# szemenyeim/DynEnv

Measured on AMD Instinct MI355X. Metric: agent-steps/s, higher is better.
Workload: dtype f64

## Files before the change

dynenv_amd/csrc/driving_dev.h:

```cpp
#pragma once
#include "dev_common.h"

#define DRV_MAXA 10
#define DRV_MAXP 20
#define DRV_MAXO 20
#define DRV_NB 32
#define DRV_NS 24
#define DRV_SLOT_PED 10
#define DRV_SLOT_OBST 30
#define DRV_SLOT_BLD 50
#define DRV_W 1700.0
#define DRV_H 1000.0
#define DRV_MAX_TIME 6000
#define DRV_TIME_DIFF 10
#define DRV_LANE_ROWS 8

enum { BF_PX = 0, BF_PY, BF_VX, BF_VY, BF_ANG, BF_W, BF_VBX, BF_VBY, BF_WB, BF_COUNT };
enum { CF_DIRX = 0, CF_DIRY, CF_PREVX, CF_PREVY, CF_GOALX, CF_GOALY, CF_COUNT };
enum { EI_ELAPSED = 0, EI_ALLFIN, EI_NPED, EI_NOBST, EI_EPISODE, EI_OCC, EI_ERR, EI_PAD,
       EI_N_FAST, EI_N_QUIET, EI_N_CONTACT, EI_N_SLOTS,
       EI_N_WHY_CAND, EI_N_WHY_MOVING, EI_N_WHY_INERT, EI_N_STEADY, EI_N_LIGHT,
       EI_N_SPLIT,
       EI_DEFER_OBS,
       EI_COUNT };
// ... 3 lines not shown
#define CARF_TYPE(f) ((f)&3)
#define CARF_TEAM(f) (((f) >> 2) & 3)
#define CARF_PACK(type, team, fin, crashed, fric, lp) \
  ((type) | ((team) << 2) | ((fin) << 4) | ((crashed) << 5) | ((fric) << 6) | ((lp) << 8))
#define PEDF_PACK(road, side, dead, crossing, begin, speed) \
  ((road) | ((side) << 1) | ((dead) << 2) | ((crossing) << 3) | ((begin) << 4) | ((speed) << 8))

struct DrvRoad {
  int nLanes;
  double width, length, dirAngle, followDist;
  double cosDir0;
  V2 p0, p1, dir, normal;
  V2 walk[2][2];
};

struct DrvConst {
  DrvRoad roads[2];
  float laneRows[DRV_LANE_ROWS * 5];
  double carMass[4], carInertia[4], carHx[4], carHy[4], carPower[4];
  double pedMass, pedInertia;
  double turnCos[2], turnSin[2];
};

struct PvIn {
  double px, py, ang;
  double ox, oy;
  double gx, gy;
  int flags;
};

struct DrvState {
  int E, A, obs_dim, pad0;
  uint64_t seed;
  int env_id_offset, pad1;
  double* body;
  double* carx;
  int* flags;
  int* aux;
  double* obst;
  int* envi;
  double* epr;
  int* s_pair;
  int* s_meta;
  uint32_t* s_hash;
  double* s_imp;
  int* lastcand;
  int* iso;
  int* iso_done;
  unsigned* iso_hw;
  int* pvq;
  int pv_par;
  int tick, iso_on;
  int tick_src;
};
#ifndef DRV_ISO_MAX
#define DRV_ISO_MAX 192
#endif
#ifndef DRV_ISO_MIN_E
#define DRV_ISO_MIN_E 3072
#endif
#define DRV_ISO_LIST 256
#define DRV_ISO_HDR 16
#define DRV_ISO_WORDS (DRV_ISO_HDR + 3 * DRV_ISO_LIST)
#define DRV_ISO_COOLDOWN 64
#define DRV_ISO_G0 256
#define DRV_ISO_GSPAN 256
#define DRV_ISO_GROUPS 1024
// ... 1 lines not shown
```

dynenv_amd/csrc/driving_kernels.hip:

```cpp
#include "driving_dev.h"

__constant__ DrvConst C;

#include "driving_host.h"

struct DrvMailbox {
  double p1x[DRV_NS][2], p1y[DRV_NS][2], p2x[DRV_NS][2], p2y[DRV_NS][2], nx[DRV_NS], ny[DRV_NS];
  int hash[DRV_NS][2], count[DRV_NS], flag[DRV_NS];
};
struct DrvObsStage {
  float carRow[DRV_MAXA][8];
  float goal[DRV_MAXA][2];
  float shared[DRV_MAXO * 4 + DRV_MAXP * 2 + DRV_LANE_ROWS * 5];
};
#ifdef DRV_PROFILE
#define DRV_PROF(...) __VA_ARGS__
#else
#define DRV_PROF(...)
#endif
#define DRV_CLIST 128
struct __align__(16) DrvLds {
  double px[DRV_NB], py[DRV_NB], vx[DRV_NB], vy[DRV_NB], ang[DRV_NB], w[DRV_NB], vbx[DRV_NB], vby[DRV_NB], wb[DRV_NB];
  double minv[DRV_NB], iinv[DRV_NB];
  double rc[16], rs[16], rotAng[16];
  double dirx[16], diry[16], prevx[16], prevy[16], goalx[16], goaly[16];
  double cosRel0[16];
  double dprev[16];
  double cmass[16], cpower[16], chx[16], chy[16];
  double aabb[DRV_MAXA][4];
  int flags[DRV_NB], moving[DRV_NB];
  double ox[DRV_MAXO], oy[DRV_MAXO];
  int s_pair[DRV_NS], s_meta[DRV_NS], s_hash0[DRV_NS], s_hash1[DRV_NS];
  double s_jn0[DRV_NS], s_jt0[DRV_NS], s_jn1[DRV_NS], s_jt1[DRV_NS];
  double rewAcc[16], posAcc[16];
  int lastCand[64];
  int stepErr;
  unsigned char act[16];
  int still[DRV_NB];
  unsigned short clist[DRV_CLIST];
  int clistN;
  int sLvMeta;
  unsigned long long sActive;
  unsigned char sLevel[DRV_NS];
  union {
    DrvMailbox mb;
    DrvObsStage ob;
  } u;
};

static_assert(sizeof(DrvLds) <= 10240, "16 one-wave workgroups per CU - one residency round of 4096 environments on 256 CUs - need <= 160 KB / 16 of LDS each");
__shared__ DrvLds g_L;


#define CF_FIN(f) (((f) >> 4) & 1)
#define CF_CRASHED(f) (((f) >> 5) & 1)
#define CF_FRIC(f) (((f) >> 6) & 1)
#define CF_LP(f) (((f) >> 8) & 7)
#define CF_SET_LP(f, lp) (((f) & ~(7 << 8)) | ((lp) << 8))
#define CF_CRASH_BITS ((1 << 4) | (1 << 5) | (1 << 6))
#define PF_ROAD(f) ((f)&1)
#define PF_SIDE(f) (((f) >> 1) & 1)
#define PF_DEAD(f) (((f) >> 2) & 1)
#define PF_CROSSING(f) (((f) >> 3) & 1)
#define PF_BEGIN(f) (((f) >> 4) & 1)
#define PF_SPEED(f) (((f) >> 8) & 15)

#define DRV_COS_PI_2 6.123233995736766e-17
template <int R>
struct RoadK;
template <>
struct RoadK<0> {
  static constexpr double p0x = 875.0, p0y = 0.0, dirx = 0.0, diry = 1.0, lat = 2.0 * 35.0 + 5.0, length = 1000.0;
  static constexpr double dirAngle = 1.5707963267948966, cosDir0 = DRV_COS_PI_2, nx = -1.0, ny = DRV_COS_PI_2;
};
// ... 556 lines not shown
      apply_impulse(a, vneg(jj), r1[c]);
      apply_impulse(b, jj, r2[c]);
    }
  }
}

DE_DEV bool arb_apply_bias_only(BodyV& a, BodyV& b, V2 n, const V2* r1, const V2* r2, const double* nMass, const double* bias,
                                double* jBias, int count) {
  bool changed = false;
#define DRV_BIAS_PASS(c)                                              \
  {                                                                   \
    double vbn = bias_rel_n(a, b, r1[c], r2[c], n);                   \
    double jbnOld = jBias[c];                                         \
    jBias[c] = dms_acc_clamp0(bias[c] - vbn, nMass[c], jbnOld);       \
    changed |= jBias[c] != jbnOld;                                    \
    V2 jb = vmul(n, jBias[c] - jbnOld);                               \
    apply_bias_impulse(a, vneg(jb), r1[c]);                           \
    apply_bias_impulse(b, jb, r2[c]);                                 \
  }
  DRV_BIAS_PASS(0)
  if (count > 1) DRV_BIAS_PASS(1)
#undef DRV_BIAS_PASS
  return changed;
}
DE_DEV bool arb_is_bias_only(const BodyV& a, const BodyV& b, const double* jn, const double* jt, const double* bounce, int count) {
  long long z = __double_as_longlong(a.v.x) | __double_as_longlong(a.v.y) | __double_as_longlong(a.w) |
                __double_as_longlong(b.v.x) | __double_as_longlong(b.v.y) | __double_as_longlong(b.w);
  bool ok = true;
#pragma unroll
  for (int c = 0; c < 2; ++c)
    if (c == 0 || count > 1) { z |= __double_as_longlong(jn[c]) | __double_as_longlong(jt[c]); ok = ok && bounce[c] == 0.0; }
  return ok && z == 0ll;
}
DE_DEV void body_load_bias(const DrvLds& L, int idx, BodyV& b) {
  if (idx < DRV_SLOT_OBST) { b.vb = v2(L.vbx[idx], L.vby[idx]); b.wb = L.wb[idx]; }
}
DE_DEV void body_store_bias(DrvLds& L, int idx, const BodyV& b) {
  if (idx < DRV_SLOT_OBST) { L.vbx[idx] = b.vb.x; L.vby[idx] = b.vb.y; L.wb[idx] = b.wb; }
}
#define DRV_ZERO_SLOT 30
#define DRV_SINK_SLOT 31
static_assert(DRV_SLOT_OBST == DRV_ZERO_SLOT && DRV_NB == 32, "body slots 30 and 31 are free");
DE_DEV int body_rd(int idx) { return idx < DRV_SLOT_OBST ? idx : DRV_ZERO_SLOT; }
DE_DEV int body_wr(int idx) { return idx < DRV_SLOT_OBST ? idx : DRV_SINK_SLOT; }

struct DrvSplitRet { double jn0, jn1, jb0, jb1, jt0, jt1; int pk, pair, bits; };
DE_OOL DrvSplitRet drv_solve_general_split(int lane, int myLevel_, int bodyAB, int lvl_, double nMass0, double nMass1, double bias0, double bias1,
                                           double bounce0, double bounce1, double jn0, double jn1, double jt0, double jt1, int pk, int pair,
                                           int bits3) {
  DrvLds& L = g_L;
  DrvMailbox& M = L.u.mb;
  int code = ((pk >> 30) & 1) | (((pk >> 8) & 0xFF) << 1) | (myLevel_ << 8);
  const int maxLevel = (int)(signed char)(uniform_i(lvl_) & 0xFF), period = uniform_i(lvl_) >> 8;
  const bool biasLane = lane >= 32;
  const int sl = lane & 31;
  code = lane_read_i(code, sl); bodyAB = lane_read_i(bodyAB, sl);
  nMass0 = lane_read_d(nMass0, sl); nMass1 = lane_read_d(nMass1, sl);
  bias0 = lane_read_d(bias0, sl); bias1 = lane_read_d(bias1, sl);
  const bool active = (code & 1) != 0 && sl < DRV_NS;
  const int count = (code >> 1) & 3, myLevel = code >> 8;
  const int bodyA = bodyAB & 0xFF, bodyB = bodyAB >> 8;
  const double nM[2] = {nMass0, nMass1};
  const double cq[2] = {biasLane ? bias0 : bounce0, biasLane ? bias1 : bounce1};
  double acc[2] = {biasLane ? 0.0 : jn0, biasLane ? 0.0 : jn1};
  V2 n = v2(0.0, 0.0), r1[2], r2[2];
  r1[0] = r1[1] = r2[0] = r2[1] = v2(0.0, 0.0);
  BodyV a, b;
  a.p = b.p = a.v = b.v = a.vb = b.vb = v2(0.0, 0.0); a.w = b.w = a.wb = b.wb = a.minv = b.minv = a.iinv = b.iinv = 0.0;
  if (active) {
    body_load(L, bodyA, a);
    body_load(L, bodyB, b);
    r1[0] = vsub(v2(M.p1x[sl][0], M.p1y[sl][0]), a.p);
    r2[0] = vsub(v2(M.p2x[sl][0], M.p2y[sl][0]), b.p);
    if (count > 1) {
      r1[1] = vsub(v2(M.p1x[sl][1], M.p1y[sl][1]), a.p);
      r2[1] = vsub(v2(M.p2x[sl][1], M.p2y[sl][1]), b.p);
    }
    n = v2(M.nx[sl], M.ny[sl]);
  }
  double* const fX = biasLane ? L.vbx : L.vx;
// ... 8 lines not shown
  {                                                                                         \
    const V2 vr = relative_velocity(a, b, r1[q], r2[q]);                                    \
    const double vn = vdot_f(vr, n);                                                        \
    const double t0 = cq[q] + (biasLane ? -vn : vn);                                        \
    const double old = acc[q];                                                              \
    acc[q] = dms_acc_clamp0(biasLane ? t0 : -t0, nM[q], old);                               \
    const double dj = acc[q] - old;                                                         \
    const V2 jr = vrotate_f(n, v2(dj, 0.0));                                                \
    const V2 jl = vmul(n, dj);                                                              \
    const V2 jj = biasLane ? jl : jr;                                                       \
    apply_impulse(a, vneg(jj), r1[q]);                                                      \
    apply_impulse(b, jj, r2[q]);                                                            \
  }
  for (int t = 0; t < nSteps; ++t) {
    if (active && t == due && passes < 10) {
      a.v = v2(fX[ra], fY[ra]); a.w = fW[ra];
      b.v = v2(fX[rb], fY[rb]); b.w = fW[rb];
      DRV_SPLIT_PASS(0)
      if (count > 1) DRV_SPLIT_PASS(1)
      fX[wa] = a.v.x; fY[wa] = a.v.y; fW[wa] = a.w;
      fX[wb_] = b.v.x; fY[wb_] = b.v.y; fW[wb_] = b.w;
      due += period; ++passes;
    }
    __syncthreads();
  }
#undef DRV_SPLIT_PASS
  DrvSplitRet r;
  r.jt0 = jt0; r.jt1 = jt1; r.pk = pk; r.pair = pair; r.bits = bits3;
  r.jn0 = acc[0]; r.jn1 = acc[1];
  r.jb0 = lane_read_d(acc[0], (lane + 32) & 63); r.jb1 = lane_read_d(acc[1], (lane + 32) & 63);
  return r;
}

DRV_PROF(__device__ unsigned long long g_dbgw[4096 * 12];)
DRV_PROF(__device__ unsigned long long g_dbgp[4096 * 8];)
DRV_PROF(__device__ unsigned long long g_dbgr[16];)
DRV_PROF(__device__ unsigned long long g_dbgl[4096 * 8];)
DRV_PROF(__device__ unsigned long long g_dbgs[4096 * 8];)
DRV_PROF(DE_DEV int prof_any(int v) { const uint64_t m = wave_ballot(v != 0); return m ? bcast_i(v, __builtin_ctzll(m)) : 0; })
#ifndef DRV_CONTACT_INLINE
#define DRV_CONTACT_INLINE __forceinline__
#endif

DE_OOL int drv_prestep_solve(int lane, int nCarPed, int pk, int a_pair, int bodyA, int bodyB, int myLevel,
                                             int maxLevel_, int anyActive_, double jn0, double jn1, double jt0, double jt1) {
  DrvLds& L = g_L;
  DrvMailbox& M = L.u.mb;
  int a_state = pk & 0xFF;
  int a_count = (pk >> 8) & 0xFF, a_age = (pk >> 16) & 0xFF;
  bool touched = (pk >> 24) & 1, freeMe = (pk >> 25) & 1, hashSame = (pk >> 26) & 1, prevInert = (pk >> 27) & 1;
  bool skipped = (pk >> 28) & 1, slotOcc = (pk >> 29) & 1, active = (pk >> 30) & 1;
  const bool isCar = lane < (uniform_i(nCarPed) & 0xFF), isPed = lane >= DRV_SLOT_PED && lane < DRV_SLOT_PED + (uniform_i(nCarPed) >> 8);
  const int maxLevel = (int)(signed char)(uniform_i(maxLevel_) & 0xFF), period = uniform_i(maxLevel_) >> 8;
  const uint64_t activeMask = uniform_i(anyActive_) ? 1ull : 0ull;
DRV_PROF(const unsigned long long P0 = __builtin_amdgcn_s_memtime();)
  double jn[2] = {jn0, jn1}, jt[2] = {jt0, jt1};
  V2 n = v2(0.0, 0.0), r1[2], r2[2];
  r1[0] = r1[1] = r2[0] = r2[1] = v2(0.0, 0.0);
  double nMass[2] = {0.0, 0.0}, tMass[2] = {0.0, 0.0}, bias[2] = {0.0, 0.0}, bounce[2] = {0.0, 0.0}, jBias[2] = {0.0, 0.0};
  const double arb_e = 0.05 * 0.05, arb_u = 0.0 * 0.0;
  bool restIn = false;
  if (active) {
    BodyV a, b;
    body_load(L, bodyA, a);
    body_load(L, bodyB, b);
    restIn = a.v.x == 0.0 && a.v.y == 0.0 && a.w == 0.0 && b.v.x == 0.0 && b.v.y == 0.0 && b.w == 0.0;
    r1[0] = vsub(v2(M.p1x[lane][0], M.p1y[lane][0]), a.p);
    r2[0] = vsub(v2(M.p2x[lane][0], M.p2y[lane][0]), b.p);
    if (a_count > 1) {
      r1[1] = vsub(v2(M.p1x[lane][1], M.p1y[lane][1]), a.p);
      r2[1] = vsub(v2(M.p2x[lane][1], M.p2y[lane][1]), b.p);
    }
    n = v2(M.nx[lane], M.ny[lane]);
    V2 body_delta = vsub(b.p, a.p);
#pragma unroll
    for (int c = 0; c < 2; ++c) {
      if (c == 0 || a_count > 1) {
        nMass[c] = 1.0 / (k_scalar_body(a, r1[c], n) + k_scalar_body(b, r2[c], n));
        double dist = vdot_f(vadd(vsub(r2[c], r1[c]), body_delta), n);
        bias[c] = -DE_CONTACT_BIAS_COEF * fmin_cp(0.0, dist + DE_COLLISION_SLOP) / DE_DT;
        jBias[c] = 0.0;
        bounce[c] = vdot_f(relative_velocity(a, b, r1[c], r2[c]), n) * arb_e;
      }
    }
  }
  __syncthreads();
DRV_PROF(const unsigned long long P1 = __builtin_amdgcn_s_memtime();)

  velocity_update(L, lane, isCar, isPed);
DRV_PROF(int profMode = 0; const unsigned long long P2 = __builtin_amdgcn_s_memtime();)
  bool tookSplit = false;
  if (activeMask && maxLevel == 0) {
    __syncthreads();
    if (active) {
      BodyV a, b;
      body_load(L, bodyA, a);
      body_load(L, bodyB, b);
      if (a_state != ARB_FIRST) arb_warm_start(a, b, n, r1, r2, jn, jt, a_count);
      if (wave_ballot(!arb_is_bias_only(a, b, jn, jt, bounce, a_count)) == 0ull) {
DRV_PROF(profMode = 1;)
#pragma unroll 1
        for (int iter = 0; iter < 10; ++iter)
          if (wave_ballot(arb_apply_bias_only(a, b, n, r1, r2, nMass, bias, jBias, a_count)) == 0ull) break;
      } else {
DRV_PROF(profMode = 2;)
#pragma unroll 1
        for (int iter = 0; iter < 10; ++iter) arb_apply_impulse(a, b, n, r1, r2, nMass, tMass, bias, bounce, jBias, jn, jt, a_count, arb_u);
      }
      body_store_vel(L, bodyA, a);
      body_store_vel(L, bodyB, b);
    }
    __syncthreads();
  } else if (activeMask) {
    __syncthreads();
    for (int lv = 0; lv <= maxLevel; ++lv) {
      if (active && myLevel == lv && a_state != ARB_FIRST) {
        BodyV a, b;
        body_load(L, bodyA, a);
        body_load(L, bodyB, b);
        arb_warm_start(a, b, n, r1, r2, jn, jt, a_count);
        body_store_vel(L, bodyA, a);
        body_store_vel(L, bodyB, b);
      }
      __syncthreads();
    }
    BodyV a, b;
    bool biasOnly = true;
    if (active) {
      body_load(L, bodyA, a); body_load(L, bodyB, b);
      biasOnly = arb_is_bias_only(a, b, jn, jt, bounce, a_count);
    }
    const int nSteps = maxLevel + 1 + period * 9;
    int due = myLevel, passes = 0;
DRV_PROF(profMode = wave_ballot(!biasOnly) == 0ull ? 3 : 4;)
    if (wave_ballot(!biasOnly) == 0ull) {
      const int ra = body_rd(bodyA), rb = body_rd(bodyB), wa = body_wr(bodyA), wb_ = body_wr(bodyB);
      for (int t = 0; t < nSteps; ++t) {
        if (active && t == due && passes < 10) {
          a.vb = v2(L.vbx[ra], L.vby[ra]); a.wb = L.wb[ra];
          b.vb = v2(L.vbx[rb], L.vby[rb]); b.wb = L.wb[rb];
          arb_apply_bias_only(a, b, n, r1, r2, nMass, bias, jBias, a_count);
          L.vbx[wa] = a.vb.x; L.vby[wa] = a.vb.y; L.wb[wa] = a.wb;
          L.vbx[wb_] = b.vb.x; L.vby[wb_] = b.vb.y; L.wb[wb_] = b.wb;
          due += period; ++passes;
        }
        __syncthreads();
      }
    } else [[unlikely]] {
      const int bits3 = (restIn ? 1 : 0) | (bias[0] == 0.0 ? 2 : 0) | (bias[1] == 0.0 ? 4 : 0);
      const DrvSplitRet sr = drv_solve_general_split(lane, myLevel, bodyA | (bodyB << 8), maxLevel_, nMass[0], nMass[1], bias[0], bias[1], bounce[0],
                                                     bounce[1], jn[0], jn[1], jt[0], jt[1], pk, a_pair, bits3);
      lane = fresh_lane();
      pk = sr.pk; a_pair = sr.pair;
      a_state = pk & 0xFF; a_count = (pk >> 8) & 0xFF; a_age = (pk >> 16) & 0xFF;
      touched = (pk >> 24) & 1; freeMe = (pk >> 25) & 1; hashSame = (pk >> 26) & 1; prevInert = (pk >> 27) & 1;
      skipped = (pk >> 28) & 1; slotOcc = (pk >> 29) & 1; active = (pk >> 30) & 1;
      restIn = (sr.bits & 1) != 0;
      bias[0] = (sr.bits & 2) ? 0.0 : 1.0; bias[1] = (sr.bits & 4) ? 0.0 : 1.0;
      jn[0] = sr.jn0; jn[1] = sr.jn1; jBias[0] = sr.jb0; jBias[1] = sr.jb1; jt[0] = sr.jt0; jt[1] = sr.jt1;
      tookSplit = true;
    }
  }
DRV_PROF(const unsigned long long P3 = __builtin_amdgcn_s_memtime();)
  const bool wasNormal = a_state == ARB_NORMAL;
  if (active && a_state == ARB_FIRST) a_state = ARB_NORMAL;
  bool steady = true;
  if (slotOcc && !skipped) {
    steady = touched && !freeMe && hashSame;
    if (steady && a_state != ARB_IGNORE) {
      steady = a_state == ARB_NORMAL && wasNormal && restIn && L.s_jn0[lane] == jn[0] && L.s_jt0[lane] == jt[0] &&
               L.s_jn1[lane] == jn[1] && L.s_jt1[lane] == jt[1];
      if (steady) {
        const int i = a_pair >> 8, j = a_pair & 0xFF;
        steady = L.vx[i] == 0.0 && L.vy[i] == 0.0 && L.w[i] == 0.0;
        if (j < DRV_SLOT_OBST) steady = steady && L.vx[j] == 0.0 && L.vy[j] == 0.0 && L.w[j] == 0.0;
      }
    }
  }
  const bool allSteady = wave_ballot(!steady) == 0ull;
  bool inert = true;
  if (slotOcc && skipped) inert = prevInert;
  else if (slotOcc) {
    inert = touched && !freeMe &&
            (a_state == ARB_IGNORE ||
             (a_state == ARB_NORMAL && wasNormal && bias[0] == 0.0 && bias[1] == 0.0 && jn[0] == 0.0 && jt[0] == 0.0 &&
              jn[1] == 0.0 && jt[1] == 0.0 && jBias[0] == 0.0 && jBias[1] == 0.0));
  }
  if (slotOcc) {
    if (freeMe) L.s_pair[lane] = 0xFFFF;
    L.s_meta[lane] = a_state | (a_count << 8) | (a_age << 16) | (steady ? (1 << 24) : 0) | (inert ? (1 << 25) : 0);
    if (touched) { L.s_jn0[lane] = jn[0]; L.s_jt0[lane] = jt[0]; L.s_jn1[lane] = jn[1]; L.s_jt1[lane] = jt[1]; }
  }
  const bool allInert = wave_ballot(!inert) == 0ull;
DRV_PROF(if (lane == 0 && blockIdx.x < 4096) { unsigned long long* d = g_dbgp + blockIdx.x * 8; const unsigned long long P4 = __builtin_amdgcn_s_memtime(); d[2] += (P1 - P0) + ((P4 - P3) << 32); d[3] += (P2 - P1) + ((P3 - P2) << 32); })
  return (allInert ? 2 : 0) | (allSteady ? 4 : 0) | (tookSplit ? 8 : 0) DRV_PROF(| (prof_any(profMode) << 4));
}
struct ContactRet {
  uint64_t occ;
  int err;
};

__device__ DRV_CONTACT_INLINE ContactRet drv_contact_path(int lane, int cand, int dirty, int light, int A, int nCarPed, uint64_t occ) {
  const bool isCar = lane < A, isPed = lane >= DRV_SLOT_PED && lane < DRV_SLOT_PED + (nCarPed >> 8);
  DrvLds& L = g_L;
  int err = 0;
  asm volatile("" : "+v"(lane));
DRV_PROF(const unsigned long long T0 = __builtin_amdgcn_s_memtime();)
  DrvMailbox& M = L.u.mb;
  if (lane < DRV_NS) M.flag[lane] = 0;
  __syncthreads();
  bool lightOk = false;
  int savedN = uniform_i(L.clistN);
  int spair = lane < DRV_NS ? L.s_pair[lane] : -1;
DRV_PROF(int profCand = 0;)
#pragma unroll 1
  for (int mode = light ? 0 : 1; mode < 2; ++mode) {
  const int bits = mode == 0 ? dirty : cand;
  bool lightBad = false;
  int nCand = 0;
  if (mode == 1 && savedN >= 0) nCand = savedN;
  else {
#pragma unroll
  for (int i = 0; i < DRV_MAXA; ++i) {
    const bool c = (bits >> i) & 1;
    const uint64_t m = wave_ballot(c);
    if (c) {
      const int idx = nCand + (int)__builtin_amdgcn_mbcnt_hi((uint32_t)(m >> 32), __builtin_amdgcn_mbcnt_lo((uint32_t)m, 0u));
      if (idx < DRV_CLIST) L.clist[idx] = (unsigned short)((i << 8) | lane); else err |= 1;
    }
    nCand += __popcll(m);
  }
  savedN = mode == 1 && nCand <= DRV_CLIST ? nCand : -1;
  if (lane == 0) L.clistN = savedN;
  if (nCand > DRV_CLIST) nCand = DRV_CLIST;
  }
// ... 214 lines not shown
    myLevel = c_level;
    maxLevel = (int)(signed char)(uniform_i(c_meta) & 0xFF);
    period = uniform_i(c_meta) >> 8;
  } else if (nActive > 1) {
    if (!haveRank && nTouched > 1)
      for (uint64_t mm = touchedMask; mm; mm &= mm - 1) {
        int b = __builtin_ctzll(mm);
        int pk = bcast_i(a_pair, b);
        rank += (pk < a_pair) ? 1 : 0;
      }
    int bl = 0;
    const int bodyAB = bodyA | (bodyB << 8);
    for (int k = 0; k < nTouched; ++k) {
      uint64_t who = wave_ballot(active && rank == k);
      if (who == 0ull) continue;
      int b = __builtin_ctzll(who);
      const int ab = bcast_i(bodyAB, b), ba = ab & 0xFF, bb2 = ab >> 8;
      const int pa = ba < DRV_SLOT_OBST ? bcast_i(bl, ba) : 0, pb = bb2 < DRV_SLOT_OBST ? bcast_i(bl, bb2) : 0;
      const int la = pa & 0xFF, lb = pb & 0xFF;
      int lv = la > lb ? la : lb;
      const int fa = (pa >> 8) - 1, fb = (pb >> 8) - 1;
      const int lo = fa < 0 ? fb : (fb < 0 ? fa : (fa < fb ? fa : fb));
      if (lo >= 0 && lv - lo + 1 > period) period = lv - lo + 1;
      if (lane == b) myLevel = lv;
      if (lane == ba || lane == bb2) bl = (lv + 1) | (((bl >> 8) ? (bl >> 8) : lv + 1) << 8);
      maxLevel = lv > maxLevel ? lv : maxLevel;
    }
    if (lane < DRV_NS) L.sLevel[lane] = (unsigned char)myLevel;
    if (lane == 0) L.sLvMeta = (maxLevel & 0xFF) | (period << 8);
  }

DRV_PROF(const unsigned long long T2 = __builtin_amdgcn_s_memtime();)
DRV_PROF(if (lane == 0 && blockIdx.x < 4096) { unsigned long long* d = g_dbgs + blockIdx.x * 8; d[0] += U1 - T1; d[1] += U2 - U1; d[2] += U3 - U2; d[3] += U4 - U3; d[4] += T2 - U4; })
  const int solveBits = drv_prestep_solve(lane, nCarPed,
                                          (a_state & 0xFF) | ((a_count & 0xFF) << 8) | ((a_age & 0xFF) << 16) | (touched ? 1 << 24 : 0) | (freeMe ? 1 << 25 : 0) |
                                              (hashSame ? 1 << 26 : 0) | (prevInert ? 1 << 27 : 0) | (skipped ? 1 << 28 : 0) | (slotOcc ? 1 << 29 : 0) | (active ? 1 << 30 : 0),
                                          a_pair, bodyA, bodyB, myLevel, (maxLevel & 0xFF) | (period << 8), activeMask != 0ull ? 1 : 0, jn[0], jn[1], jt[0], jt[1]);
  occ &= ~freeMask;
DRV_PROF(const unsigned long long T3 = T2, T4 = T2, T5 = __builtin_amdgcn_s_memtime(); const int profModeW = (uniform_i(solveBits) >> 4) & 7;)
DRV_PROF(if (lane == 0 && blockIdx.x < 4096) { unsigned long long* d = g_dbgp + blockIdx.x * 8; d[0] += T1 - T0; d[1] += T2 - T1; d[2] += T3 - T2; d[3] += T4 - T3; d[4] += T5 - T4; d[5] += 1ull + (light ? (1ull << 16) : 0ull); d[6] += (unsigned long long)(maxLevel + 1) + ((unsigned long long)(maxLevel + 1) << (12 * profModeW)); d[7] += (unsigned long long)nTouched + ((unsigned long long)profCand << 16); })
  {
    ContactRet ret;
    ret.occ = occ; ret.err = err | (uniform_i(solveBits) & 6) | ((uniform_i(solveBits) & 8) << 1);
    return ret;
  }
}

DE_OOL int drv_partial_obs_fused(PvIn in, uint64_t seed, int A, int* envi, int env_id_offset, int e, int nPedObst, int elapsed,
                                 uint32_t episode, int noiseTypeAgents, double magn, float* __restrict__ obs, int budgetCycles);
#ifndef DRV_DEFER_MIN_CONTACT
#define DRV_DEFER_MIN_CONTACT 5
#endif
#ifndef DRV_PV_DEADLINE_PCT
#define DRV_PV_DEADLINE_PCT 110
#endif
#ifndef DRV_FUSED_AGENTS
#define DRV_FUSED_AGENTS 10
#endif
struct DrvLightRet {
  int cand, dirty, bits;
};
struct DrvSeedOnly { uint64_t seed; };
DE_OOL DrvLightRet drv_light_substep(int it_, int lane, int A_, int nPed_, int nObst_, int elapsed_,
                                                      uint32_t seedLo, uint32_t seedHi, uint32_t genv_, uint32_t episode_, int stateBits) {
  DrvLds& L = g_L;
DRV_PROF(const unsigned long long Q0 = __builtin_amdgcn_s_memtime();)
  const int lastCand = L.lastCand[lane];
  const int it = uniform_i(it_), A = uniform_i(A_), nPed = uniform_i(nPed_), nObst = uniform_i(nObst_), elapsed = uniform_i(elapsed_);
  const uint32_t genv = (uint32_t)uniform_i((int)genv_), episode = (uint32_t)uniform_i((int)episode_);
  DrvSeedOnly S;
// ... 277 lines not shown
#ifndef DRV_ISO_MIN
#define DRV_ISO_MIN 300000
#endif
#ifndef DRV_ISO_PCT
#define DRV_ISO_PCT 75
#endif
DE_DEV void drv_iso_report(const DrvState& S, int e, int lane, unsigned long long t0, int tick) {
  if (!S.iso_on || lane != 0) return;
  const int cycles = (int)(__builtin_amdgcn_s_memtime() - t0);
  const int buf = tick % 3, nxt = (tick + 1) % 3;
  const int slowest = S.iso[3 + buf];
  if (cycles > DRV_ISO_MIN && cycles > (slowest / 100) * DRV_ISO_PCT) atomicMax(&S.iso[3 + nxt], cycles);
  if (S.iso_on == 3) return;
  if (slowest > DRV_ISO_MIN && cycles > (slowest / 100) * DRV_ISO_PCT) {
    const int k = atomicAdd(&S.iso[nxt], 1);
    if (k < DRV_ISO_LIST) S.iso[DRV_ISO_HDR + nxt * DRV_ISO_LIST + k] = e;
  }
  __atomic_store_n(&S.iso_done[e], tick, __ATOMIC_RELAXED);
}

template <bool PARTIAL>
DE_DEV void drv_step_body(const DrvState& S, const int* __restrict__ actions, float* __restrict__ obs, double* __restrict__ rewards,
                          uint8_t* __restrict__ dones, float* __restrict__ pobs, int pvNoise, double pvMagn) {
  const unsigned long long isoT0 = __builtin_amdgcn_s_memtime();
DRV_PROF(const unsigned long long KS = isoT0;)
  DrvLds& L = g_L;
  int lane = threadIdx.x;
  const int tick = drv_launch_tick(S);
  if (!S.tick_src && blockIdx.x == 0 && lane == 0) { S.iso[13] = S.tick; S.iso[14] = S.pv_par; }
  const int e = drv_iso_assign(S, lane, tick);
  if (e < 0) return;
DRV_PROF(if (lane < 8 && e < 4096) { g_dbgp[e * 8 + lane] = 0ull; g_dbgs[e * 8 + lane] = 0ull; })
  const int A = S.A;
  int* envi = S.envi + (size_t)e * EI_COUNT;
  int elapsed = uniform_i(envi[EI_ELAPSED]);
  int allFinished = uniform_i(envi[EI_ALLFIN]);
  const int nPed = uniform_i(envi[EI_NPED]);
  const int nObst = uniform_i(envi[EI_NOBST]);
  const uint32_t episode = (uint32_t)uniform_i(envi[EI_EPISODE]);
  uint64_t occ = (uint64_t)(uint32_t)uniform_i(envi[EI_OCC]);
  if (occ != 0ull) __builtin_amdgcn_s_setprio(3);
  else if (PARTIAL) __builtin_amdgcn_s_setprio(1);
  const uint32_t genv = (uint32_t)(S.env_id_offset + e);

  const bool isCar = lane < A;
  const bool isPed = lane >= DRV_SLOT_PED && lane < DRV_SLOT_PED + nPed;
  const bool isBody = isCar || isPed;
  const int g_act0 = actions[((size_t)e * A + (isCar ? lane : 0)) * 2 + 0], g_act1 = actions[((size_t)e * A + (isCar ? lane : 0)) * 2 + 1];
  const int g_lastCand = S.lastcand[(size_t)e * 64 + lane];
  load_env(S, L, e, lane, A, nPed, nObst, occ);

  {
    int act0 = isCar ? g_act0 : 1, act1 = isCar ? g_act1 : 1;
    const bool bad = (unsigned)act0 > 2u || (unsigned)act1 > 2u;
    if (bad) { act0 = 1; act1 = 1; }
    if (lane < 16) L.act[lane] = (unsigned char)(act0 | (act1 << 2));
    const bool anyBad = wave_ballot(bad) != 0ull;
    if (lane == 0) L.stepErr = anyBad ? 2 : 0;
  }
  int finishedAt = -1;
  if (lane < 16) { L.rewAcc[lane] = 0.0; L.posAcc[lane] = 0.0; }
  bool aabbValid = false;
  L.lastCand[lane] = g_lastCand;
  if (lane == 0) { L.clistN = -1; L.sActive = ~0ull; L.sLvMeta = 0; }
  bool inertAll = (uniform_i(envi[EI_PAD]) & 1) != 0;
  bool steadyAll = (uniform_i(envi[EI_PAD]) & 2) != 0;
// ... 2 lines not shown
  __syncthreads();

DRV_PROF(const unsigned long long K0 = __builtin_amdgcn_s_memtime(); unsigned long long tPh1 = 0, tBroad = 0, tFast = 0, tCont = 0, tBook = 0;)
  bool lightOff = false;
  for (int it = 0; it < 10; ++it) {
    lane = fresh_lane();
DRV_PROF(const unsigned long long A0 = __builtin_amdgcn_s_memtime();)
    const DrvLightRet lr = drv_light_substep(it, lane, A, nPed, nObst, elapsed, (uint32_t)S.seed, (uint32_t)(S.seed >> 32), genv, episode,
                                             (vbValid ? 1 : 0) | (aabbValid ? 2 : 0));
    const int cand = lr.cand, dirty = lr.dirty;
    const bool candMoving = (lr.bits & 1) != 0, removed = (lr.bits & 2) != 0;
    aabbValid = true;
DRV_PROF(const unsigned long long A1 = A0;)
    const uint64_t anyCand = wave_ballot(cand != 0);
    const bool candChanged = wave_ballot((lr.bits & 4) != 0) != 0ull, anyMoving = wave_ballot(candMoving) != 0ull;
    if (candChanged && lane == 0) L.clistN = -1;
    const bool quiescent = inertAll && !candChanged && !anyMoving;
    const bool steadyOk = !quiescent && steadyAll && wave_ballot(removed) == 0ull;
    const bool anyDirty = wave_ballot(dirty != 0) != 0ull;
    bool replay = steadyOk && !anyDirty;
    const bool light = steadyOk && anyDirty && !lightOff;
    if (!(anyCand == 0ull && occ == 0ull) && !quiescent && !replay) { if (candChanged) nWhyCand++; else if (anyMoving) nWhyMoving++; else nWhyInert++; }

DRV_PROF(const unsigned long long A2 = __builtin_amdgcn_s_memtime(); bool tookContact = false;)
    if (anyCand == 0ull && occ == 0ull) nFast++; else if (quiescent) nQuiet++; else if (replay) nSteady++; else nContact++;
    nSlots += __popcll(occ);
    if ((anyCand == 0ull && occ == 0ull) || quiescent) {
      velocity_update_ool(A | (nPed << 8));
      if (anyCand == 0ull && occ == 0ull) steadyAll = false;
      vbValid = false;
    } else if (!replay) {
DRV_PROF(tookContact = true;)
      __builtin_amdgcn_s_setprio(3);
      ContactRet cr = drv_contact_path(lane, cand, dirty, light ? 1 : 0, A, A | (nPed << 8), occ);
      lane = fresh_lane();
      if (wave_ballot((cr.err & 1) != 0) != 0ull && lane == 0) L.stepErr |= 1;
      if (light && !(uniform_i(cr.err >> 3) & 1)) lightOff = true;
      if (uniform_i(cr.err >> 3) & 1) {
        replay = true; nLight++;
      } else {
        nSplit += uniform_i(cr.err >> 4) & 1;
        occ = uniform_u64(cr.occ);
        inertAll = (uniform_i(cr.err >> 1) & 1) != 0;
        steadyAll = (uniform_i(cr.err >> 2) & 1) != 0;
        vbValid = true;
      }
    }
    if (replay) {
      velocity_update_ool(A | (nPed << 8));
      vbValid = true;
    }
    __syncthreads();

DRV_PROF(const unsigned long long A3 = __builtin_amdgcn_s_memtime(); tPh1 += A1 - A0; tBroad += A2 - A1; if (tookContact) tCont += A3 - A2; else tFast += A3 - A2;)
    elapsed += 1;
    bool notDone = false;
    if (isCar) { int f = L.flags[lane]; notDone = !(CF_FIN(f) && !CF_CRASHED(f)); }
    const bool allFin = wave_ballot(notDone) == 0ull;
    if (!allFinished && allFin) {
      allFinished = 1;
      finishedAt = elapsed;
    }
  }
  lane = fresh_lane();
  const double teamReward = finishedAt >= 0 ? 0.0 + (double)(DRV_MAX_TIME - finishedAt) / 100.0 : 0.0;

DRV_PROF(const unsigned long long K1 = __builtin_amdgcn_s_memtime();)
  double* er = S.epr + (size_t)e * 16 + (isCar ? lane : 0);
// ... 215 lines not shown
```

dynenv_amd/csrc/driving_tu.hip:

```cpp
#include <hip/hip_runtime.h>

#include "driving_kernels.hip"
#include "driving_partial.hip"
#include "dynenv_host.h"

#define ISO_PROBE_EVERY 64
#define ISO_PAUSE_STEPS 2048

static void road_init_host(DrvRoad& r, int nLanes, double width, V2 p0, V2 p1) {
  V2 d = vsub(p1, p0);
  r.nLanes = nLanes; r.width = width; r.p0 = p0; r.p1 = p1; r.followDist = 90.0;
  r.length = vlen(d);
  r.dir = v2(d.x / r.length, d.y / r.length);
  r.normal = vrot_angle(r.dir, DM_PI / 2.0);
  r.dirAngle = dm_atan2(r.dir.y, r.dir.x);
  r.cosDir0 = dm_cos(r.dirAngle - 0.0);
  double k = (double)(nLanes + 1) * width;
  r.walk[0][0] = vadd(p0, vmul(r.normal, k)); r.walk[0][1] = vadd(p1, vmul(r.normal, k));
  r.walk[1][0] = vsub(p0, vmul(r.normal, k)); r.walk[1][1] = vsub(p1, vmul(r.normal, k));
}

static double moment_for_box(double m, double hx, double hy) {
  V2 verts[4] = {v2(hx, hy), v2(-hx, hy), v2(-hx, -hy), v2(hx, -hy)};
  double sum1 = 0.0, sum2 = 0.0;
// ... 82 lines not shown
    if (iso_clear(false, nullptr)) return DYNENV_ERR_HIP;
    HIP_OK(hipMemset(S.pvq, 0, sizeof(int) * 32));
    S.pv_par = 0;
    return 0;
  }

  int init() override {
    A = cfg.n_players > DRV_MAXA ? DRV_MAXA : cfg.n_players;
    partial = cfg.obs_type == DYNENV_OBS_PARTIAL;
    full_dim = drv_full_row(A); global_dim = 0; state_bytes = sizeof(dynenv_driving_state_t);
    obs_dim = partial ? PV_DIM : full_dim; T = 1; action_dim = 2;
    memset(&S, 0, sizeof(S));
    const size_t E = (size_t)cfg.num_envs;
    S.E = (int)E; S.A = A; S.obs_dim = full_dim; S.seed = cfg.seed; S.env_id_offset = cfg.env_id_offset;
    int rc = 0;
    rc |= alloc(&S.body, (size_t)BF_COUNT * E * DRV_NB);
    rc |= alloc(&S.carx, (size_t)CF_COUNT * E * 16);
    rc |= alloc(&S.flags, E * DRV_NB);
    rc |= alloc(&S.aux, E * DRV_NB);
    rc |= alloc(&S.obst, 2 * E * DRV_MAXO);
    rc |= alloc(&S.envi, E * EI_COUNT);
    rc |= alloc(&S.epr, 2 * E * 16);
    rc |= alloc(&S.s_pair, E * DRV_NS);
    rc |= alloc(&S.s_meta, E * DRV_NS);
    rc |= alloc(&S.s_hash, 2 * E * DRV_NS);
    rc |= alloc(&S.s_imp, 4 * E * DRV_NS);
    rc |= alloc(&S.lastcand, E * 64);
    rc |= alloc(&S.iso, DRV_ISO_WORDS, SCRATCH);
    rc |= alloc(&S.iso_done, E, SCRATCH);
    rc |= alloc(&S.iso_hw, 2 * 4 * DRV_ISO_GROUPS, SCRATCH);
    rc |= alloc(&S.pvq, 32 + 2 * (size_t)S.E, SCRATCH);
    if (rc) return DYNENV_ERR_HIP;
    err_array = S.envi; err_stride = EI_COUNT; err_index = EI_ERR;
    {
      hipDeviceProp_t prop;
      S.iso_on = 0;
      if (hipGetDeviceProperties(&prop, cfg.device_id) == hipSuccess)
      {
        const bool dev256 = prop.multiProcessorCount * 4 == DRV_ISO_GROUPS, off = getenv("DYNENV_NO_ISOLATION") != nullptr;
        const int isoMinE = getenv("DYNENV_ISO_MIN_E") ? atoi(getenv("DYNENV_ISO_MIN_E")) : DRV_ISO_MIN_E;
        S.iso_on = off || !dev256 ? 0 : ((int)E > isoMinE && E <= 4 * DRV_ISO_GROUPS ? (partial ? 0 : 1) : (E > 4 * DRV_ISO_GROUPS ? 2 : 0));
        if (!off && S.iso_on == 0 && partial) S.iso_on = 3;
      }
      if (iso_reset()) return DYNENV_ERR_HIP;
      iso_cfg = S.iso_on;
      if (S.iso_on == 1) {
        if (hipHostMalloc((void**)&iso_seen, sizeof(int), hipHostMallocDefault) != hipSuccess) return fail(DYNENV_ERR_HIP, "hipHostMalloc");
        *iso_seen = 0;
      }
    }
    DrvConst c;
    build_consts(c);
    if (!drv_literals_ok(c)) return fail(DYNENV_ERR_HIP, "internal: RoadK / CarK literals differ from the computed constants");
    hipError_t e = hipMemcpyToSymbol(HIP_SYMBOL(C), &c, sizeof(c));
    if (e != hipSuccess) return fail(DYNENV_ERR_HIP, hipGetErrorString(e));
    return DYNENV_OK;
  }

  void layout(dynenv_layout_t& L) const override {
    L.steps_per_episode = DRV_MAX_TIME / 10;
    if (!partial) { drv_full_row(A, &L); return; }
    const int off[6] = {0, PV_OFF_CARS, PV_OFF_OBST, PV_OFF_PEDS, PV_OFF_LANES, PV_DIM - 4};
    const int rows[6] = {1, PV_CAP_CARS, PV_CAP_OBST, PV_CAP_PEDS, PV_CAP_LANES, 1}, feat[6] = {9, 7, 6, 2, 4, 4};
    row_blocks(&L, 6, rows, feat, off);
  }

// ... 200 lines not shown
```

Before: 260.8 million.

## Skip identity warm-start passes and move general split solve out of prestep

Adds a check that skips the level-by-level warm-start loop, with its per-level barriers, when all bodies and accumulated impulses are zero. It also skips the steady-state body-velocity recheck when the rest path already proved it. The rare general split solve is moved out of the prestep function into a separate tail call, so the common path is meant to be leaner on registers. An environment variable can turn the fast path off. The cost is more code and a more complex control flow.

```diff
diff --git a/dynenv_amd/csrc/driving_dev.h b/dynenv_amd/csrc/driving_dev.h
--- a/dynenv_amd/csrc/driving_dev.h
+++ b/dynenv_amd/csrc/driving_dev.h
@@ -59,7 +59,8 @@
 struct DrvState {
   int E, A, obs_dim, pad0;
   uint64_t seed;
-  int env_id_offset, pad1;
+  int env_id_offset;
+  int no_fastpath;
   double* body;
   double* carx;
   int* flags;
diff --git a/dynenv_amd/csrc/driving_kernels.hip b/dynenv_amd/csrc/driving_kernels.hip
--- a/dynenv_amd/csrc/driving_kernels.hip
+++ b/dynenv_amd/csrc/driving_kernels.hip
@@ -40,6 +40,7 @@
   unsigned short clist[DRV_CLIST];
   int clistN;
   int sLvMeta;
+  int noFast;
   unsigned long long sActive;
   unsigned char sLevel[DRV_NS];
   union {
@@ -662,6 +663,12 @@
     if (c == 0 || count > 1) { z |= __double_as_longlong(jn[c]) | __double_as_longlong(jt[c]); ok = ok && bounce[c] == 0.0; }
   return ok && z == 0ll;
 }
+DE_DEV bool arb_warm_start_is_identity(const BodyV& a, const BodyV& b, const double* jn, const double* jt) {
+  const long long z = __double_as_longlong(a.v.x) | __double_as_longlong(a.v.y) | __double_as_longlong(a.w) | __double_as_longlong(b.v.x) |
+                      __double_as_longlong(b.v.y) | __double_as_longlong(b.w) | __double_as_longlong(jn[0]) | __double_as_longlong(jt[0]) |
+                      __double_as_longlong(jn[1]) | __double_as_longlong(jt[1]);
+  return z == 0ll;
+}
 DE_DEV void body_load_bias(const DrvLds& L, int idx, BodyV& b) {
   if (idx < DRV_SLOT_OBST) { b.vb = v2(L.vbx[idx], L.vby[idx]); b.wb = L.wb[idx]; }
 }
@@ -675,7 +682,7 @@
 DE_DEV int body_wr(int idx) { return idx < DRV_SLOT_OBST ? idx : DRV_SINK_SLOT; }
 
 struct DrvSplitRet { double jn0, jn1, jb0, jb1, jt0, jt1; int pk, pair, bits; };
-DE_OOL DrvSplitRet drv_solve_general_split(int lane, int myLevel_, int bodyAB, int lvl_, double nMass0, double nMass1, double bias0, double bias1,
+DE_DEV DrvSplitRet drv_solve_general_split(int lane, int myLevel_, int bodyAB, int lvl_, double nMass0, double nMass1, double bias0, double bias1,
                                            double bounce0, double bounce1, double jn0, double jn1, double jt0, double jt1, int pk, int pair,
                                            int bits3) {
   DrvLds& L = g_L;
@@ -750,6 +757,42 @@
   return r;
 }
 
+DE_DEV int drv_slot_verdicts(DrvLds& L, int lane, int a_state, int a_count, int a_age, bool touched, bool freeMe, bool hashSame, bool prevInert,
+                             bool skipped, bool slotOcc, bool active, int a_pair, bool restIn, bool bias0Zero, bool bias1Zero, const double* jn,
+                             const double* jt, const double* jBias, bool restKnown) {
+  const bool wasNormal = a_state == ARB_NORMAL;
+  if (active && a_state == ARB_FIRST) a_state = ARB_NORMAL;
+  bool steady = true;
+  if (slotOcc && !skipped) {
+    steady = touched && !freeMe && hashSame;
+    if (steady && a_state != ARB_IGNORE) {
+      steady = a_state == ARB_NORMAL && wasNormal && restIn && L.s_jn0[lane] == jn[0] && L.s_jt0[lane] == jt[0] &&
+               L.s_jn1[lane] == jn[1] && L.s_jt1[lane] == jt[1];
+      if (steady && !restKnown) {
+        const int i = a_pair >> 8, j = a_pair & 0xFF;
+        steady = L.vx[i] == 0.0 && L.vy[i] == 0.0 && L.w[i] == 0.0;
+        if (j < DRV_SLOT_OBST) steady = steady && L.vx[j] == 0.0 && L.vy[j] == 0.0 && L.w[j] == 0.0;
+      }
+    }
+  }
+  const bool allSteady = wave_ballot(!steady) == 0ull;
+  bool inert = true;
+  if (slotOcc && skipped) inert = prevInert;
+  else if (slotOcc) {
+    inert = touched && !freeMe &&
+            (a_state == ARB_IGNORE ||
+             (a_state == ARB_NORMAL && wasNormal && bias0Zero && bias1Zero && jn[0] == 0.0 && jt[0] == 0.0 &&
+              jn[1] == 0.0 && jt[1] == 0.0 && jBias[0] == 0.0 && jBias[1] == 0.0));
+  }
+  if (slotOcc) {
+    if (freeMe) L.s_pair[lane] = 0xFFFF;
+    L.s_meta[lane] = a_state | (a_count << 8) | (a_age << 16) | (steady ? (1 << 24) : 0) | (inert ? (1 << 25) : 0);
+    if (touched) { L.s_jn0[lane] = jn[0]; L.s_jt0[lane] = jt[0]; L.s_jn1[lane] = jn[1]; L.s_jt1[lane] = jt[1]; }
+  }
+  const bool allInert = wave_ballot(!inert) == 0ull;
+  return (allInert ? 2 : 0) | (allSteady ? 4 : 0);
+}
+
 DRV_PROF(__device__ unsigned long long g_dbgw[4096 * 12];)
 DRV_PROF(__device__ unsigned long long g_dbgp[4096 * 8];)
 DRV_PROF(__device__ unsigned long long g_dbgr[16];)
@@ -760,8 +803,14 @@
 #define DRV_CONTACT_INLINE __forceinline__
 #endif
 
+DE_OOL DrvSplitRet drv_solve_general_split_ool(int lane, int myLevel, int bodyAB, int lvl, double nMass0, double nMass1, double bias0, double bias1, double bounce0,
+                                               double bounce1, double jn0, double jn1, double jt0, double jt1, int pk, int pair, int bits3) {
+  return drv_solve_general_split(lane, myLevel, bodyAB, lvl, nMass0, nMass1, bias0, bias1, bounce0, bounce1, jn0, jn1, jt0, jt1, pk, pair, bits3);
+}
+struct DrvSplitArgs { double nMass0, nMass1, bias0, bias1, bounce0, bounce1, jn0, jn1, jt0, jt1; int myLevel, bodyAB, lvl, pk, pair, bits3; };
+template <bool LEAF>
 DE_OOL int drv_prestep_solve(int lane, int nCarPed, int pk, int a_pair, int bodyA, int bodyB, int myLevel,
-                                             int maxLevel_, int anyActive_, double jn0, double jn1, double jt0, double jt1) {
+                                             int maxLevel_, int anyActive_, double jn0, double jn1, double jt0, double jt1, DrvSplitArgs* rare) {
   DrvLds& L = g_L;
   DrvMailbox& M = L.u.mb;
   int a_state = pk & 0xFF;
@@ -772,6 +821,7 @@
   const int maxLevel = (int)(signed char)(uniform_i(maxLevel_) & 0xFF), period = uniform_i(maxLevel_) >> 8;
   const uint64_t activeMask = uniform_i(anyActive_) ? 1ull : 0ull;
 DRV_PROF(const unsigned long long P0 = __builtin_amdgcn_s_memtime();)
+  const int noFast_ = L.noFast;
   double jn[2] = {jn0, jn1}, jt[2] = {jt0, jt1};
   V2 n = v2(0.0, 0.0), r1[2], r2[2];
   r1[0] = r1[1] = r2[0] = r2[1] = v2(0.0, 0.0);
@@ -806,17 +856,23 @@
 DRV_PROF(const unsigned long long P1 = __builtin_amdgcn_s_memtime();)
 
   velocity_update(L, lane, isCar, isPed);
-DRV_PROF(int profMode = 0; const unsigned long long P2 = __builtin_amdgcn_s_memtime();)
+DRV_PROF(int profMode = 0; int profWarm = 0; const unsigned long long P2 = __builtin_amdgcn_s_memtime(); unsigned long long PW = P2;)
+  const bool noFast = uniform_i(noFast_) != 0;
   bool tookSplit = false;
+  bool restOut = false;
   if (activeMask && maxLevel == 0) {
     __syncthreads();
     if (active) {
       BodyV a, b;
       body_load(L, bodyA, a);
       body_load(L, bodyB, b);
-      if (a_state != ARB_FIRST) arb_warm_start(a, b, n, r1, r2, jn, jt, a_count);
+      const bool warm = a_state != ARB_FIRST && (noFast || !arb_warm_start_is_identity(a, b, jn, jt));
+DRV_PROF(profWarm = wave_ballot(warm) != 0ull ? 1 : 0;)
+      if (warm) arb_warm_start(a, b, n, r1, r2, jn, jt, a_count);
+DRV_PROF(PW = __builtin_amdgcn_s_memtime();)
       if (wave_ballot(!arb_is_bias_only(a, b, jn, jt, bounce, a_count)) == 0ull) {
 DRV_PROF(profMode = 1;)
+        restOut = true;
 #pragma unroll 1
         for (int iter = 0; iter < 10; ++iter)
           if (wave_ballot(arb_apply_bias_only(a, b, n, r1, r2, nMass, bias, jBias, a_count)) == 0ull) break;
@@ -831,27 +887,35 @@
     __syncthreads();
   } else if (activeMask) {
     __syncthreads();
-    for (int lv = 0; lv <= maxLevel; ++lv) {
-      if (active && myLevel == lv && a_state != ARB_FIRST) {
-        BodyV a, b;
-        body_load(L, bodyA, a);
-        body_load(L, bodyB, b);
-        arb_warm_start(a, b, n, r1, r2, jn, jt, a_count);
-        body_store_vel(L, bodyA, a);
-        body_store_vel(L, bodyB, b);
-      }
-      __syncthreads();
-    }
     BodyV a, b;
-    bool biasOnly = true;
+    bool warm = false;
     if (active) {
       body_load(L, bodyA, a); body_load(L, bodyB, b);
-      biasOnly = arb_is_bias_only(a, b, jn, jt, bounce, a_count);
-    }
+      warm = a_state != ARB_FIRST && !arb_warm_start_is_identity(a, b, jn, jt);
+    }
+    if (noFast || wave_ballot(warm) != 0ull) {
+DRV_PROF(profWarm = 1;)
+      for (int lv = 0; lv <= maxLevel; ++lv) {
+        if (active && myLevel == lv && a_state != ARB_FIRST) {
+          BodyV wa, wb;
+          body_load(L, bodyA, wa);
+          body_load(L, bodyB, wb);
+          arb_warm_start(wa, wb, n, r1, r2, jn, jt, a_count);
+          body_store_vel(L, bodyA, wa);
+          body_store_vel(L, bodyB, wb);
+        }
+        __syncthreads();
+      }
+      if (active) { body_load(L, bodyA, a); body_load(L, bodyB, b); }
+    }
+DRV_PROF(PW = __builtin_amdgcn_s_memtime();)
+    bool biasOnly = true;
+    if (active) biasOnly = arb_is_bias_only(a, b, jn, jt, bounce, a_count);
     const int nSteps = maxLevel + 1 + period * 9;
     int due = myLevel, passes = 0;
 DRV_PROF(profMode = wave_ballot(!biasOnly) == 0ull ? 3 : 4;)
     if (wave_ballot(!biasOnly) == 0ull) {
+      restOut = true;
       const int ra = body_rd(bodyA), rb = body_rd(bodyB), wa = body_wr(bodyA), wb_ = body_wr(bodyB);
       for (int t = 0; t < nSteps; ++t) {
         if (active && t == due && passes < 10) {
@@ -865,60 +929,56 @@
         __syncthreads();
       }
     } else [[unlikely]] {
-      const int bits3 = (restIn ? 1 : 0) | (bias[0] == 0.0 ? 2 : 0) | (bias[1] == 0.0 ? 4 : 0);
-      const DrvSplitRet sr = drv_solve_general_split(lane, myLevel, bodyA | (bodyB << 8), maxLevel_, nMass[0], nMass[1], bias[0], bias[1], bounce[0],
-                                                     bounce[1], jn[0], jn[1], jt[0], jt[1], pk, a_pair, bits3);
-      lane = fresh_lane();
-      pk = sr.pk; a_pair = sr.pair;
-      a_state = pk & 0xFF; a_count = (pk >> 8) & 0xFF; a_age = (pk >> 16) & 0xFF;
-      touched = (pk >> 24) & 1; freeMe = (pk >> 25) & 1; hashSame = (pk >> 26) & 1; prevInert = (pk >> 27) & 1;
-      skipped = (pk >> 28) & 1; slotOcc = (pk >> 29) & 1; active = (pk >> 30) & 1;
-      restIn = (sr.bits & 1) != 0;
-      bias[0] = (sr.bits & 2) ? 0.0 : 1.0; bias[1] = (sr.bits & 4) ? 0.0 : 1.0;
-      jn[0] = sr.jn0; jn[1] = sr.jn1; jBias[0] = sr.jb0; jBias[1] = sr.jb1; jt[0] = sr.jt0; jt[1] = sr.jt1;
-      tookSplit = true;
+      if constexpr (LEAF) {
+        rare->myLevel = myLevel; rare->bodyAB = bodyA | (bodyB << 8); rare->lvl = maxLevel_; rare->pk = pk; rare->pair = a_pair;
+        rare->bits3 = (restIn ? 1 : 0) | (bias[0] == 0.0 ? 2 : 0) | (bias[1] == 0.0 ? 4 : 0);
+        rare->nMass0 = nMass[0]; rare->nMass1 = nMass[1]; rare->bias0 = bias[0]; rare->bias1 = bias[1]; rare->bounce0 = bounce[0]; rare->bounce1 = bounce[1];
+        rare->jn0 = jn[0]; rare->jn1 = jn[1]; rare->jt0 = jt[0]; rare->jt1 = jt[1];
+DRV_PROF(if (lane == 0 && blockIdx.x < 4096) { unsigned long long* d = g_dbgp + blockIdx.x * 8; const unsigned long long P3 = __builtin_amdgcn_s_memtime(); d[2] += P1 - P0; d[3] += (P2 - P1) + ((P3 - P2) << 32); unsigned long long* ds = g_dbgs + blockIdx.x * 8; ds[5] += 1ull; ds[7] += PW - P2; })
+        return 8 DRV_PROF(| (4 << 4));
+      } else {
+        const int bits3 = (restIn ? 1 : 0) | (bias[0] == 0.0 ? 2 : 0) | (bias[1] == 0.0 ? 4 : 0);
+        const DrvSplitRet sr = drv_solve_general_split_ool(lane, myLevel, bodyA | (bodyB << 8), maxLevel_, nMass[0], nMass[1], bias[0], bias[1], bounce[0],
+                                                           bounce[1], jn[0], jn[1], jt[0], jt[1], pk, a_pair, bits3);
+        lane = fresh_lane();
+        pk = sr.pk; a_pair = sr.pair;
+        a_state = pk & 0xFF; a_count = (pk >> 8) & 0xFF; a_age = (pk >> 16) & 0xFF;
+        touched = (pk >> 24) & 1; freeMe = (pk >> 25) & 1; hashSame = (pk >> 26) & 1; prevInert = (pk >> 27) & 1;
+        skipped = (pk >> 28) & 1; slotOcc = (pk >> 29) & 1; active = (pk >> 30) & 1;
+        restIn = (sr.bits & 1) != 0;
+        bias[0] = (sr.bits & 2) ? 0.0 : 1.0; bias[1] = (sr.bits & 4) ? 0.0 : 1.0;
+        jn[0] = sr.jn0; jn[1] = sr.jn1; jBias[0] = sr.jb0; jBias[1] = sr.jb1; jt[0] = sr.jt0; jt[1] = sr.jt1;
+        tookSplit = true;
+      }
     }
   }
 DRV_PROF(const unsigned long long P3 = __builtin_amdgcn_s_memtime();)
-  const bool wasNormal = a_state == ARB_NORMAL;
-  if (active && a_state == ARB_FIRST) a_state = ARB_NORMAL;
-  bool steady = true;
-  if (slotOcc && !skipped) {
-    steady = touched && !freeMe && hashSame;
-    if (steady && a_state != ARB_IGNORE) {
-      steady = a_state == ARB_NORMAL && wasNormal && restIn && L.s_jn0[lane] == jn[0] && L.s_jt0[lane] == jt[0] &&
-               L.s_jn1[lane] == jn[1] && L.s_jt1[lane] == jt[1];
-      if (steady) {
-        const int i = a_pair >> 8, j = a_pair & 0xFF;
-        steady = L.vx[i] == 0.0 && L.vy[i] == 0.0 && L.w[i] == 0.0;
-        if (j < DRV_SLOT_OBST) steady = steady && L.vx[j] == 0.0 && L.vy[j] == 0.0 && L.w[j] == 0.0;
-      }
-    }
-  }
-  const bool allSteady = wave_ballot(!steady) == 0ull;
-  bool inert = true;
-  if (slotOcc && skipped) inert = prevInert;
-  else if (slotOcc) {
-    inert = touched && !freeMe &&
-            (a_state == ARB_IGNORE ||
-             (a_state == ARB_NORMAL && wasNormal && bias[0] == 0.0 && bias[1] == 0.0 && jn[0] == 0.0 && jt[0] == 0.0 &&
-              jn[1] == 0.0 && jt[1] == 0.0 && jBias[0] == 0.0 && jBias[1] == 0.0));
-  }
-  if (slotOcc) {
-    if (freeMe) L.s_pair[lane] = 0xFFFF;
-    L.s_meta[lane] = a_state | (a_count << 8) | (a_age << 16) | (steady ? (1 << 24) : 0) | (inert ? (1 << 25) : 0);
-    if (touched) { L.s_jn0[lane] = jn[0]; L.s_jt0[lane] = jt[0]; L.s_jn1[lane] = jn[1]; L.s_jt1[lane] = jt[1]; }
-  }
-  const bool allInert = wave_ballot(!inert) == 0ull;
-DRV_PROF(if (lane == 0 && blockIdx.x < 4096) { unsigned long long* d = g_dbgp + blockIdx.x * 8; const unsigned long long P4 = __builtin_amdgcn_s_memtime(); d[2] += (P1 - P0) + ((P4 - P3) << 32); d[3] += (P2 - P1) + ((P3 - P2) << 32); })
-  return (allInert ? 2 : 0) | (allSteady ? 4 : 0) | (tookSplit ? 8 : 0) DRV_PROF(| (prof_any(profMode) << 4));
+  const int verdicts = drv_slot_verdicts(L, lane, a_state, a_count, a_age, touched, freeMe, hashSame, prevInert, skipped, slotOcc, active, a_pair, restIn,
+                                         bias[0] == 0.0, bias[1] == 0.0, jn, jt, jBias, restOut && !noFast);
+DRV_PROF(const int profWarmAny = prof_any(profWarm); { const uint64_t pm = wave_ballot(PW != P2); if (pm) { const int pl = __builtin_ctzll(pm); PW = ((unsigned long long)(unsigned)bcast_i((int)(PW >> 32), pl) << 32) | (unsigned)bcast_i((int)PW, pl); } })
+DRV_PROF(if (lane == 0 && blockIdx.x < 4096) { unsigned long long* d = g_dbgp + blockIdx.x * 8; const unsigned long long P4 = __builtin_amdgcn_s_memtime(); d[2] += (P1 - P0) + ((P4 - P3) << 32); d[3] += (P2 - P1) + ((P3 - P2) << 32); if (activeMask) { unsigned long long* ds = g_dbgs + blockIdx.x * 8; ds[5] += 1ull; ds[6] += profWarmAny ? 0ull : 1ull; ds[7] += PW - P2; } })
+  return verdicts | (tookSplit ? 8 : 0) DRV_PROF(| (prof_any(profMode) << 4));
+}
+DE_OOL int drv_general_tail(int lane, const DrvSplitArgs* q) {
+DRV_PROF(const unsigned long long G0 = __builtin_amdgcn_s_memtime();)
+  const DrvSplitRet sr = drv_solve_general_split(lane, q->myLevel, q->bodyAB, q->lvl, q->nMass0, q->nMass1, q->bias0, q->bias1, q->bounce0, q->bounce1,
+                                                 q->jn0, q->jn1, q->jt0, q->jt1, q->pk, q->pair, q->bits3);
+DRV_PROF(const unsigned long long G1 = __builtin_amdgcn_s_memtime();)
+  const int pk = sr.pk;
+  const double jn[2] = {sr.jn0, sr.jn1}, jt[2] = {sr.jt0, sr.jt1}, jBias[2] = {sr.jb0, sr.jb1};
+  const int verdicts = drv_slot_verdicts(g_L, lane, pk & 0xFF, (pk >> 8) & 0xFF, (pk >> 16) & 0xFF, (pk >> 24) & 1, (pk >> 25) & 1, (pk >> 26) & 1, (pk >> 27) & 1,
+                                         (pk >> 28) & 1, (pk >> 29) & 1, (pk >> 30) & 1, sr.pair, (sr.bits & 1) != 0, (sr.bits & 2) != 0, (sr.bits & 4) != 0, jn, jt,
+                                         jBias, false);
+DRV_PROF(if (lane == 0 && blockIdx.x < 4096) { unsigned long long* d = g_dbgp + blockIdx.x * 8; const unsigned long long G2 = __builtin_amdgcn_s_memtime(); d[2] += (G2 - G1) << 32; d[3] += (G1 - G0) << 32; d[4] += G2 - G0; })
+  return verdicts | 8;
 }
 struct ContactRet {
   uint64_t occ;
   int err;
 };
 
-__device__ DRV_CONTACT_INLINE ContactRet drv_contact_path(int lane, int cand, int dirty, int light, int A, int nCarPed, uint64_t occ) {
+template <bool LEAF>
+__device__ DRV_CONTACT_INLINE ContactRet drv_contact_path(int lane, int cand, int dirty, int light, int A, int nCarPed, uint64_t occ, DrvSplitArgs* rare) {
   const bool isCar = lane < A, isPed = lane >= DRV_SLOT_PED && lane < DRV_SLOT_PED + (nCarPed >> 8);
   DrvLds& L = g_L;
   int err = 0;
@@ -1199,10 +1259,10 @@
 
 DRV_PROF(const unsigned long long T2 = __builtin_amdgcn_s_memtime();)
 DRV_PROF(if (lane == 0 && blockIdx.x < 4096) { unsigned long long* d = g_dbgs + blockIdx.x * 8; d[0] += U1 - T1; d[1] += U2 - U1; d[2] += U3 - U2; d[3] += U4 - U3; d[4] += T2 - U4; })
-  const int solveBits = drv_prestep_solve(lane, nCarPed,
+  const int solveBits = drv_prestep_solve<LEAF>(lane, nCarPed,
                                           (a_state & 0xFF) | ((a_count & 0xFF) << 8) | ((a_age & 0xFF) << 16) | (touched ? 1 << 24 : 0) | (freeMe ? 1 << 25 : 0) |
                                               (hashSame ? 1 << 26 : 0) | (prevInert ? 1 << 27 : 0) | (skipped ? 1 << 28 : 0) | (slotOcc ? 1 << 29 : 0) | (active ? 1 << 30 : 0),
-                                          a_pair, bodyA, bodyB, myLevel, (maxLevel & 0xFF) | (period << 8), activeMask != 0ull ? 1 : 0, jn[0], jn[1], jt[0], jt[1]);
+                                          a_pair, bodyA, bodyB, myLevel, (maxLevel & 0xFF) | (period << 8), activeMask != 0ull ? 1 : 0, jn[0], jn[1], jt[0], jt[1], rare);
   occ &= ~freeMask;
 DRV_PROF(const unsigned long long T3 = T2, T4 = T2, T5 = __builtin_amdgcn_s_memtime(); const int profModeW = (uniform_i(solveBits) >> 4) & 7;)
 DRV_PROF(if (lane == 0 && blockIdx.x < 4096) { unsigned long long* d = g_dbgp + blockIdx.x * 8; d[0] += T1 - T0; d[1] += T2 - T1; d[2] += T3 - T2; d[3] += T4 - T3; d[4] += T5 - T4; d[5] += 1ull + (light ? (1ull << 16) : 0ull); d[6] += (unsigned long long)(maxLevel + 1) + ((unsigned long long)(maxLevel + 1) << (12 * profModeW)); d[7] += (unsigned long long)nTouched + ((unsigned long long)profCand << 16); })
@@ -1546,6 +1606,7 @@
   if (e < 0) return;
 DRV_PROF(if (lane < 8 && e < 4096) { g_dbgp[e * 8 + lane] = 0ull; g_dbgs[e * 8 + lane] = 0ull; })
   const int A = S.A;
+  L.noFast = S.no_fastpath;
   int* envi = S.envi + (size_t)e * EI_COUNT;
   int elapsed = uniform_i(envi[EI_ELAPSED]);
   int allFinished = uniform_i(envi[EI_ALLFIN]);
@@ -1614,8 +1675,11 @@
     } else if (!replay) {
 DRV_PROF(tookContact = true;)
       __builtin_amdgcn_s_setprio(3);
-      ContactRet cr = drv_contact_path(lane, cand, dirty, light ? 1 : 0, A, A | (nPed << 8), occ);
+      DrvSplitArgs rare;
+      ContactRet cr = drv_contact_path<!PARTIAL>(lane, cand, dirty, light ? 1 : 0, A, A | (nPed << 8), occ, &rare);
       lane = fresh_lane();
+      if constexpr (!PARTIAL)
+        if (uniform_i(cr.err >> 4) & 1) [[unlikely]] cr.err = (cr.err & ~6) | (drv_general_tail(lane, &rare) & 6);
       if (wave_ballot((cr.err & 1) != 0) != 0ull && lane == 0) L.stepErr |= 1;
       if (light && !(uniform_i(cr.err >> 3) & 1)) lightOff = true;
       if (uniform_i(cr.err >> 3) & 1) {
diff --git a/dynenv_amd/csrc/driving_tu.hip b/dynenv_amd/csrc/driving_tu.hip
--- a/dynenv_amd/csrc/driving_tu.hip
+++ b/dynenv_amd/csrc/driving_tu.hip
@@ -138,6 +138,7 @@
     rc |= alloc(&S.pvq, 32 + 2 * (size_t)S.E, SCRATCH);
     if (rc) return DYNENV_ERR_HIP;
     err_array = S.envi; err_stride = EI_COUNT; err_index = EI_ERR;
+    S.no_fastpath = getenv("DYNENV_NO_CONTACT_FASTPATH") != nullptr ? 1 : 0;
     {
       hipDeviceProp_t prop;
       S.iso_on = 0;
```

New measurement: 262.9 million (median of 6 runs). No clear change (+0.8%).
